# silence-tang/GaussianIP

Measured on AMD Instinct MI355X. Metric: raster_fwd_bwd_mpix_per_s, higher is better.
Workload: dtype f32; 1 GPU; BASELINE.json configs[1]: 100000 Gaussians (synthetic human surface, SMPL-X-style init), 1024x1024, 4 views per optimizer step, raster forward+backward; gaussians=100000, height=1024, width=1024, prewarm_steps=0, repeats=11, full=False, sh_degree=0, dist_world_size=1, gpus_visible=1, parallelism=1 GPU

## Files before the change

### gaussianip_amd/_lib.py

```python
import ctypes
import os

_HERE = os.path.dirname(os.path.abspath(__file__))
LIB_DIR = os.path.join(_HERE, "lib")

GIP_MAX_VIEWS = 16
GIP_RECORD_BYTES = 64
GIP_PARTIAL_FLOATS = 12
GIP_OK = 0

_vp = ctypes.c_void_p


class GipRasterConfig(ctypes.Structure):
    _fields_ = [("P", ctypes.c_int32), ("V", ctypes.c_int32), ("H", ctypes.c_int32), ("W", ctypes.c_int32),
                ("sh_degree", ctypes.c_int32), ("sh_coeffs", ctypes.c_int32), ("prefiltered", ctypes.c_int32),
                ("debug", ctypes.c_int32), ("scale_modifier", ctypes.c_float),
                ("tanfovx", ctypes.c_float * GIP_MAX_VIEWS), ("tanfovy", ctypes.c_float * GIP_MAX_VIEWS),
                ("capacity", ctypes.c_uint64), ("exact_lists", ctypes.c_int32), ("forward_only", ctypes.c_int32),
                ("sh_scalar", ctypes.c_int32), ("antialiasing", ctypes.c_int32)]


class GipRasterInputs(ctypes.Structure):
    _fields_ = [(n, _vp) for n in ("means3D", "shs", "colors_precomp", "opacities", "scales", "rotations",
# ... 33 lines not shown

call_counts = {}


class _Counted:

    def __init__(self, lib):
        self._lib = lib
        self._wrapped = {}

    def __getattr__(self, name):
        w = self._wrapped.get(name)
        if w is None:
            fn = getattr(self._lib, name)

            names = (name, name.replace("_buckets", "")) if name.startswith("gip_raster_") and "_buckets" in name else (name,)

            def w(*args, _fn=fn, _names=names):
                for n in _names:
                    call_counts[n] = call_counts.get(n, 0) + 1
                return _fn(*args)
            self._wrapped[name] = w
        return w


def raster_lib():
    global _raster
    if _raster is None:
        path = os.path.join(LIB_DIR, os.environ.get("GIP_RASTER_LIB", "libgip_raster.so"))
        if not os.path.exists(path):
            raise _missing("libgip_raster.so")
# ... 20 lines not shown
        lib.gip_raster_backward_profiled.argtypes = lib.gip_raster_backward.argtypes + [ctypes.POINTER(ctypes.c_float)]
        _u32 = ctypes.c_uint32
        lib.gip_raster_state_bytes_buckets.restype = ctypes.c_size_t
        lib.gip_raster_state_bytes_buckets.argtypes = [ctypes.POINTER(GipRasterConfig), _u32]
        lib.gip_raster_state_layout_buckets.restype = ctypes.c_int
        lib.gip_raster_state_layout_buckets.argtypes = [ctypes.POINTER(GipRasterConfig), _u32, ctypes.POINTER(GipRasterStateLayout),
                                                        ctypes.POINTER(ctypes.c_size_t)]
        lib.gip_raster_forward_buckets.restype = ctypes.c_int
        lib.gip_raster_forward_buckets.argtypes = lib.gip_raster_forward.argtypes + [_u32]
        lib.gip_raster_backward_buckets.restype = ctypes.c_int
        lib.gip_raster_backward_buckets.argtypes = lib.gip_raster_backward.argtypes + [_u32]
        lib.gip_raster_forward_buckets_profiled.restype = ctypes.c_int
        lib.gip_raster_forward_buckets_profiled.argtypes = lib.gip_raster_forward.argtypes + [_u32, ctypes.POINTER(ctypes.c_float)]
        lib.gip_raster_backward_buckets_profiled.restype = ctypes.c_int
        lib.gip_raster_backward_buckets_profiled.argtypes = lib.gip_raster_backward.argtypes + [_u32, ctypes.POINTER(ctypes.c_float)]
        lib.gip_raster_read_header.restype = ctypes.c_int
        lib.gip_raster_read_header.argtypes = [_vp, _vp, _vp]
        lib.gip_raster_mark_visible.restype = ctypes.c_int
        lib.gip_raster_mark_visible.argtypes = [ctypes.c_int32, _vp, _vp, _vp, _vp, _vp]
        _raster = _Counted(lib)
    return _raster


def knn_lib():
    global _knn
    if _knn is None:
        path = os.path.join(LIB_DIR, "libgip_knn.so")
        if not os.path.exists(path):
            raise _missing("libgip_knn.so")
        lib = ctypes.CDLL(path)
# ... 379 lines not shown
        lib.gip_softmax_rows_backward_f16.argtypes = [_vp, _vp, ctypes.c_int64, ctypes.c_int32, ctypes.c_float, _vp]
        lib.gip_scale_cast_f16.restype = ctypes.c_int
        lib.gip_scale_cast_f16.argtypes = [_vp, _vp, ctypes.c_float, _vp, ctypes.c_int64, _vp]
        _nn = _Counted(lib)
    return _nn


def status_string(rc):
    return raster_lib().gip_status_string(int(rc)).decode()


RASTER_SYMBOLS = ["gip_abi_version", "gip_status_string", "gip_raster_state_bytes", "gip_raster_scratch_bytes",
                  "gip_raster_state_layout", "gip_raster_forward", "gip_raster_backward", "gip_raster_read_header",
                  "gip_raster_mark_visible", "gip_raster_forward_profiled", "gip_raster_backward_profiled",
                  "gip_raster_state_bytes_buckets", "gip_raster_state_layout_buckets", "gip_raster_forward_buckets",
                  "gip_raster_backward_buckets", "gip_raster_forward_buckets_profiled", "gip_raster_backward_buckets_profiled"]
FIELD_SYMBOLS = ["gip_field_workspace_size", "gip_density_field", "gip_surface_count", "gip_surface_emit"]
SAMPLE_SYMBOLS = ["gip_field_sample_workspace_size", "gip_field_sample"]
TEXTURE_SYMBOLS = ["gip_texture_bake_workspace_size", "gip_texture_bake"]
TEXTURE_PROJECT_SYMBOLS = ["gip_texture_project"]
MESH_SYMBOLS = ["gip_mesh_raster_workspace_size", "gip_mesh_rasterize", "gip_mesh_interpolate", "gip_mesh_interpolate_backward",
                "gip_mesh_texture", "gip_mesh_texture_backward", "gip_mesh_shade", "gip_mesh_shade_backward"]
MESH_GRAD_SYMBOLS = ["gip_mesh_rasterize_backward", "gip_mesh_interpolate_backward_rast", "gip_mesh_shade_backward_rast", "gip_mesh_antialias",
                     "gip_mesh_antialias_backward"]
MESH_MIP_SYMBOLS = ["gip_mesh_rast_db", "gip_mesh_interpolate_da", "gip_mesh_interpolate_da_backward", "gip_mesh_mip_levels",
                    "gip_mesh_mip_build", "gip_mesh_mip_fold", "gip_mesh_texture_mip", "gip_mesh_texture_mip_backward"]
MESH_CLEAN_SYMBOLS = ["gip_mesh_components_rounds", "gip_mesh_component_stats", "gip_mesh_cluster_keys", "gip_mesh_cluster_count",
                      "gip_mesh_cluster_place"]
MESH_GEOM_SYMBOLS = ["gip_mesh_geometry_workspace_size", "gip_mesh_vertex_normals", "gip_mesh_vertex_normals_backward",
                     "gip_mesh_laplacian_loss", "gip_mesh_laplacian_loss_backward", "gip_mesh_normal_consistency",
                     "gip_mesh_normal_consistency_backward"]
# ... 10 lines not shown
```

### gaussianip_amd/csrc/api.hip

```cpp
#include <string.h>

#include "gip_internal.h"

static inline size_t align256(size_t x) { return (x + 255) & ~(size_t)255; }

static_assert(offsetof(GipRasterConfig, antialiasing) == 188 && sizeof(GipRasterConfig) == 192, "GipRasterConfig layout");

static bool sh_mfma_path(const GipRasterConfig* c) { return c->sh_coeffs > 0 && c->sh_degree >= 1 && c->V >= 2 && !c->sh_scalar; }

static bool valid_config(const GipRasterConfig* c) {
  if (!c) return false;
  if (c->P < 0 || c->V < 1 || c->V > GIP_MAX_VIEWS || c->H < 1 || c->W < 1) return false;
  if (c->sh_degree < 0 || c->sh_degree > 3) return false;
  if (c->capacity < 1 || c->capacity > 0xfffffff0ull) return false;
  if ((c->H + GIP_TILE - 1) / GIP_TILE > 0xffff || (c->W + GIP_TILE - 1) / GIP_TILE > 0xffff) return false;
  return true;
}

extern "C" int gip_abi_version(void) { return GIP_ABI_VERSION; }

extern "C" const char* gip_status_string(int status) {
  switch (status) {
    case GIP_OK: return "ok";
    case GIP_ERR_BAD_ARGUMENT: return "bad argument (null pointer, or not exactly one of shs/colors_precomp and scales+rotations/cov3D_precomp)";
// ... 96 lines not shown
  p.tile_cursor = (uint32_t*)(b + L.tile_cursor);
  p.tile_count_b = (uint32_t*)(b + L.tile_count_b);
  p.inst_slot = (uint32_t*)(b + L.inst_slot);
  p.block_sums = (uint32_t*)(b + L.block_sums);
  p.block_offset = (uint32_t*)(b + L.block_offset);
  p.keys = (unsigned long long*)(b + (bucket_keys ? bucket_keys : L.keys));
  p.n_contrib = (uint32_t*)(b + L.n_contrib);
  p.final_T = (float*)(b + L.final_T);
  p.tile_order = (uint32_t*)(b + L.tile_order);
  p.seg_start = (uint32_t*)(b + L.seg_start);
  p.ckpt_start = (uint32_t*)(b + L.ckpt_start);
  p.seg_tile = (uint32_t*)(b + L.seg_tile);
  p.checkpoints = (float*)(b + L.checkpoints);
  p.sh_colors = (float*)(b + L.sh_colors);
  p.host_header = nullptr;
  return p;
}

static int prepare(const GipRasterConfig* cfg, const GipRasterInputs* in, void* state, size_t state_bytes, uint32_t bucket_stride,
                   GipRasterStateLayout* L, GipKernelParams* kp, GipStatePtrs* st) {
  size_t bucket_keys = 0;
  if (gip_raster_state_layout_buckets(cfg, bucket_stride, L, &bucket_keys) != GIP_OK) return GIP_ERR_BAD_ARGUMENT;
  if (state_bytes < L->total) return GIP_ERR_BUFFER_TOO_SMALL;
  fill_params(cfg, *L, kp);
  kp->bucket_stride = bucket_stride;
  if (!in->shs) kp->sh_mfma = 0;
  *st = state_ptrs(state, *L, bucket_stride ? bucket_keys : 0);
  return GIP_OK;
}

// ... 39 lines not shown
    if (!ok || hipStreamSynchronize(s) != hipSuccess) rc = GIP_ERR_HIP;
    for (int i = 0; i < GIP_NUM_STAGES; i++) {
      if (rc == GIP_OK && used[i]) {
        float ms = 0.f;
        if (hipEventElapsedTime(&ms, ev[2 * i], ev[2 * i + 1]) != hipSuccess) rc = GIP_ERR_HIP;
        out[i] = ms;
      }
    }
    for (int i = 0; i < created; i++) (void)hipEventDestroy(ev[i]);
    return rc;
  }
};
}

static int forward_impl(const GipRasterConfig* cfg, const GipRasterInputs* in, const GipRasterOutputs* out,
                        void* state, size_t state_bytes, void* stream, float* times, uint32_t bucket_stride) {
  if (!valid_config(cfg)) return cfg && (cfg->V > GIP_MAX_VIEWS || cfg->sh_degree > 3) ? GIP_ERR_UNSUPPORTED : GIP_ERR_BAD_ARGUMENT;
  int rc = check_inputs(cfg, in);
  if (rc != GIP_OK) return rc;
  if (!out || !out->color || !out->radii || !out->depth || !out->alpha || !state) return GIP_ERR_BAD_ARGUMENT;
  GipRasterStateLayout L;
  GipKernelParams kp;
  GipStatePtrs st;
  rc = prepare(cfg, in, state, state_bytes, bucket_stride, &L, &kp, &st);
  if (rc != GIP_OK) return rc;
  st.host_header = out->host_header;
  hipStream_t s = (hipStream_t)stream;
  StageTimer tm(s, times);

  tm.begin(GIP_STAGE_CLEAR);
  HIP_TRY(hipMemsetAsync((char*)state + L.header, 0, L.tile_start - L.header, s));
  tm.end(GIP_STAGE_CLEAR);
  if (cfg->P > 0) {
    tm.begin(GIP_STAGE_PREPROCESS);
    if (kp.sh_mfma) gip_launch_sh_forward_mfma(kp, *in, st.sh_colors, s);
    gip_launch_preprocess(kp, *in, out->radii, st, s);
    tm.end(GIP_STAGE_PREPROCESS);
    LAUNCH_CHECK();
  }
  tm.begin(GIP_STAGE_SCAN);
  gip_launch_scan(kp, st, s);
  tm.end(GIP_STAGE_SCAN);
  LAUNCH_CHECK();
  if (cfg->P > 0) {
    if (!bucket_stride) {
      tm.begin(GIP_STAGE_SCATTER);
      gip_launch_scatter(kp, st, s);
// ... 13 lines not shown
}

extern "C" int gip_raster_forward(const GipRasterConfig* cfg, const GipRasterInputs* in, const GipRasterOutputs* out,
                                  void* state, size_t state_bytes, void* stream) {
  return forward_impl(cfg, in, out, state, state_bytes, stream, nullptr, 0);
}
extern "C" int gip_raster_forward_buckets(const GipRasterConfig* cfg, const GipRasterInputs* in, const GipRasterOutputs* out,
                                          void* state, size_t state_bytes, void* stream, uint32_t bucket_stride) {
  return forward_impl(cfg, in, out, state, state_bytes, stream, nullptr, bucket_stride);
}
extern "C" int gip_raster_forward_buckets_profiled(const GipRasterConfig* cfg, const GipRasterInputs* in, const GipRasterOutputs* out,
                                                   void* state, size_t state_bytes, void* stream, uint32_t bucket_stride,
                                                   float* times_ms) {
  if (!times_ms) return GIP_ERR_BAD_ARGUMENT;
  return forward_impl(cfg, in, out, state, state_bytes, stream, times_ms, bucket_stride);
}
extern "C" int gip_raster_forward_profiled(const GipRasterConfig* cfg, const GipRasterInputs* in, const GipRasterOutputs* out,
                                           void* state, size_t state_bytes, void* stream, float* times_ms) {
  if (!times_ms) return GIP_ERR_BAD_ARGUMENT;
  return forward_impl(cfg, in, out, state, state_bytes, stream, times_ms, 0);
}

static int backward_impl(const GipRasterConfig* cfg, const GipRasterInputs* in, const GipRasterGradsIn* gin,
                         const void* state, size_t state_bytes, void* scratch, size_t scratch_bytes,
                         const GipRasterGradsOut* gout, void* stream, float* times, uint32_t bucket_stride) {
  if (!valid_config(cfg)) return GIP_ERR_BAD_ARGUMENT;
  int rc = check_inputs(cfg, in);
  if (rc != GIP_OK) return rc;
  if (!gin || !gin->alpha || !gin->color || !gin->depth || !gout || !state || !scratch) return GIP_ERR_BAD_ARGUMENT;
  if (cfg->forward_only) return GIP_ERR_BAD_ARGUMENT;
// ... 60 lines not shown
```

### gaussianip_amd/csrc/binning.hip

```cpp
#include "gip_internal.h"
#include "tile_sort_assign.h"

#define SCAN_THREADS 1024
#define SCAN_WAVES (SCAN_THREADS / 64)
#define SCAN_CHUNK SCAN_THREADS
#define SCAN_FIN 32

__device__ __forceinline__ uint32_t nseg_of(uint32_t count) { return (count + GIP_SEGMENT - 1) / GIP_SEGMENT; }

#define ORDER_CLASSES 6
__device__ __forceinline__ int class_of(uint32_t c) {
  return c >= 2048 ? 0 : c >= 1024 ? 1 : c >= 512 ? 2 : c >= 128 ? 3 : c >= 1 ? 4 : 5;
}

__device__ __forceinline__ uint32_t block_excl_scan(uint32_t v, uint32_t* s_w, uint32_t* total) {
  const int lane = threadIdx.x & 63, wave = threadIdx.x >> 6;
  const uint32_t incl = gip_wave_incl_scan_u32(v);
  __syncthreads();
  if (lane == 63) s_w[wave] = incl;
  __syncthreads();
  uint32_t base = 0, tot = 0;
#pragma unroll
  for (int w = 0; w < SCAN_WAVES; w++) { const uint32_t x = s_w[w]; base += w < wave ? x : 0u; tot += x; }
  *total = tot;
  return base + incl - v;
}

__device__ __forceinline__ uint32_t wave_sum_u32(uint32_t v) {
#pragma unroll
  for (int d = 32; d >= 1; d >>= 1) v += (uint32_t)__shfl_xor((int)v, d, 64);
  return v;
}

__global__ void __launch_bounds__(SCAN_THREADS)
gip_scan_kernel(GipKernelParams kp, const uint32_t* __restrict__ tile_count, const uint32_t* __restrict__ tile_count_b,
                uint32_t* __restrict__ tile_start,
                uint32_t* __restrict__ seg_start, uint32_t* __restrict__ ckpt_start,
                const uint32_t* __restrict__ block_sums, uint32_t* __restrict__ block_offset,
                uint32_t* __restrict__ tile_order, GipRasterHeader* __restrict__ header, uint32_t* __restrict__ host_header,
                uint32_t* __restrict__ inst_offset) {
  __shared__ uint32_t s_w[SCAN_WAVES];
  __shared__ uint32_t s_acc[2][3 + ORDER_CLASSES];
  __shared__ uint32_t s_max;
  __shared__ uint32_t s_cls[ORDER_CLASSES][SCAN_WAVES];
  const int n = kp.V * kp.T;
  const int n_chunks = (n + SCAN_CHUNK - 1) / SCAN_CHUNK;
  const int tid = threadIdx.x, lane = tid & 63, wave = tid >> 6;
  const int nb_chunks = kp.V * kp.nblk > 0 ? (kp.V * kp.nblk + SCAN_CHUNK - 1) / SCAN_CHUNK : 1;
  if ((int)blockIdx.x >= n_chunks + nb_chunks) {
    __shared__ uint32_t s_fin[SCAN_FIN];
    const int nb = kp.V * kp.nblk;
    const int j0 = ((int)blockIdx.x - n_chunks - nb_chunks) * SCAN_FIN;
    uint32_t before = 0;
    for (int i = tid; i < j0; i += SCAN_THREADS) before += block_sums[i];
    before = wave_sum_u32(before);
    if (tid == 0) s_max = 0u;
    __syncthreads();
// ... 22 lines not shown
      uint32_t v8[8];
#pragma unroll
      for (int u = 0; u < 8; u++) { const int i = i0 + u * SCAN_THREADS; v8[u] = i < c0 ? block_sums[i] : 0u; }
#pragma unroll
      for (int u = 0; u < 8; u++) before += v8[u];
    }
    before = wave_sum_u32(before);
    if (tid == 0) s_max = 0u;
    __syncthreads();
    if (lane == 0) atomicAdd(&s_max, before);
    __syncthreads();
    const uint32_t base = s_max;
    const int i = c0 + tid;
    const uint32_t v = i < nb ? block_sums[i] : 0u;
    uint32_t total;
    const uint32_t e = block_excl_scan(v, s_w, &total);
    if (i < nb) block_offset[i] = base + e;
    if (c0 + SCAN_CHUNK >= nb && tid == 0) block_offset[nb] = base + total;
    return;
  }
  const int chunk0 = (int)blockIdx.x * SCAN_CHUNK;
  if (tid < 2 * (3 + ORDER_CLASSES)) (&s_acc[0][0])[tid] = 0u;
  if (tid == 0) s_max = 0u;
  __syncthreads();
  uint32_t b_c = 0, b_s = 0, b_k = 0, t_c = 0, t_s = 0, t_k = 0, mx = 0;
  uint32_t b_cls[ORDER_CLASSES], t_cls[ORDER_CLASSES];
#pragma unroll
  for (int c = 0; c < ORDER_CLASSES; c++) { b_cls[c] = 0; t_cls[c] = 0; }
  for (int i0 = wave * 64; i0 < n; i0 += 8 * SCAN_THREADS) {
    uint32_t va[8], vb[8];
#pragma unroll
    for (int u = 0; u < 8; u++) {
      const int i = i0 + u * SCAN_THREADS + lane;
      va[u] = i < n ? tile_count[i] : 0u;
      vb[u] = i < n ? tile_count_b[i] : 0u;
    }
#pragma unroll
    for (int u = 0; u < 8; u++) {
      const int g0 = i0 + u * SCAN_THREADS;
      if (g0 >= n) break;
      const int i = g0 + lane;
      const uint32_t c = va[u] + vb[u], a = nseg_of(c), k = a ? a - 1 : 0;
      const int cls = i < n ? class_of(c) : -1;
      const bool before = g0 < chunk0;
      t_c += c; t_s += a; t_k += k;
      mx = c > mx ? c : mx;
      if (before) { b_c += c; b_s += a; b_k += k; }
#pragma unroll
      for (int q = 0; q < ORDER_CLASSES; q++) {
        const uint32_t m = (uint32_t)__popcll(__ballot(cls == q));
        t_cls[q] += m;
        if (before) b_cls[q] += m;
      }
    }
  }
  b_c = wave_sum_u32(b_c); b_s = wave_sum_u32(b_s); b_k = wave_sum_u32(b_k);
  t_c = wave_sum_u32(t_c); t_s = wave_sum_u32(t_s); t_k = wave_sum_u32(t_k);
  mx = gip_wave_max_u32(mx);
  if (lane == 0) {
    atomicAdd(&s_acc[0][0], b_c); atomicAdd(&s_acc[0][1], b_s); atomicAdd(&s_acc[0][2], b_k);
    atomicAdd(&s_acc[1][0], t_c); atomicAdd(&s_acc[1][1], t_s); atomicAdd(&s_acc[1][2], t_k);
#pragma unroll
    for (int q = 0; q < ORDER_CLASSES; q++) { atomicAdd(&s_acc[0][3 + q], b_cls[q]); atomicAdd(&s_acc[1][3 + q], t_cls[q]); }
    atomicMax(&s_max, mx);
  }
  __syncthreads();
  const int i = chunk0 + tid;
  uint32_t c = 0;
  if (i < n) c = tile_count[i] + tile_count_b[i];
  const uint32_t a = nseg_of(c), k = a ? a - 1 : 0;
  uint32_t tot;
  const uint32_t e_c = block_excl_scan(c, s_w, &tot);
  const uint32_t e_s = block_excl_scan(a, s_w, &tot);
  const uint32_t e_k = block_excl_scan(k, s_w, &tot);
  if (i < n) {
    tile_start[i] = s_acc[0][0] + e_c;
    seg_start[i] = s_acc[0][1] + e_s;
    ckpt_start[i] = s_acc[0][2] + e_k;
  }
  const int cls = i < n ? class_of(c) : -1;
  uint32_t rank = 0;
#pragma unroll
  for (int q = 0; q < ORDER_CLASSES; q++) {
    const unsigned long long m = __ballot(cls == q);
    if (cls == q) rank = (uint32_t)__popcll(m & ((1ull << lane) - 1ull));
    if (lane == 0) s_cls[q][wave] = (uint32_t)__popcll(m);
  }
  __syncthreads();
  if (cls >= 0) {
    uint32_t pos = rank + s_acc[0][3 + cls];
#pragma unroll
    for (int q = 0; q < ORDER_CLASSES; q++) pos += q < cls ? s_acc[1][3 + q] : 0u;
    for (int w = 0; w < wave; w++) pos += s_cls[cls][w];
    tile_order[pos] = (uint32_t)i;
  }
  if (blockIdx.x == 0 && tid == 0) {
    const uint32_t total = s_acc[1][0];
    tile_start[n] = total; seg_start[n] = s_acc[1][1]; ckpt_start[n] = s_acc[1][2];
    const uint32_t n0 = s_acc[1][3], n1 = s_acc[1][4], n2 = s_acc[1][5], n3 = s_acc[1][6], n4 = s_acc[1][7];
    header->class_end[1] = n0;
    header->class_end[2] = n0 + n1;
    header->class_end[0] = n0 + n1 + n2;
    header->class_end[3] = n0 + n1 + n2 + n3 + n4;
    header->abi_version = GIP_ABI_VERSION;
    header->num_rendered = total;
    const uint32_t over = (total > kp.capacity || (kp.bucket_stride && s_max > kp.bucket_stride)) ? 1u : 0u;
    header->overflow = over;
    header->max_tile_count = s_max;
    header->reserved[0] = kp.bucket_stride;
    header->num_segments = s_acc[1][1];
    header->num_checkpoints = s_acc[1][2];
    if (host_header) {
      host_header[0] = GIP_ABI_VERSION; host_header[1] = total;
      host_header[2] = over; host_header[3] = s_max; host_header[4] = kp.bucket_stride;
    }
  }
}

void gip_launch_scan(const GipKernelParams& kp, GipStatePtrs st, hipStream_t s) {
  const int n = kp.V * kp.T, nb = kp.V * kp.nblk;
  const int n_chunks = (n + SCAN_CHUNK - 1) / SCAN_CHUNK, b_chunks = nb > 0 ? (nb + SCAN_CHUNK - 1) / SCAN_CHUNK : 1;
  const int f_chunks = kp.bucket_stride ? (nb + SCAN_FIN - 1) / SCAN_FIN : 0;
  hipLaunchKernelGGL(gip_scan_kernel, dim3(n_chunks + b_chunks + f_chunks), dim3(SCAN_THREADS), 0, s, kp, st.tile_count, st.tile_count_b, st.tile_start,
                     st.seg_start, st.ckpt_start, st.block_sums, st.block_offset, st.tile_order, st.header, st.host_header,
                     st.inst_offset);
}

__global__ void __launch_bounds__(GIP_BLOCK)
gip_scatter_kernel(GipKernelParams kp, const GipRecord* __restrict__ records, const uint32_t* __restrict__ tile_start,
                   const uint32_t* __restrict__ tile_count, uint32_t* __restrict__ tile_cursor,
                   const uint32_t* __restrict__ inst_slot, const uint32_t* __restrict__ block_offset,
                   uint32_t* __restrict__ inst_offset, unsigned long long* __restrict__ keys) {
  const int v = blockIdx.y;
  const int idx = blockIdx.x * GIP_BLOCK + threadIdx.x;
  uint32_t tiles = 0, rmin = 0, rmax = 0, dbits = 0, tmask = 0;
  if (idx < kp.P) {
    const uint4* rp = reinterpret_cast<const uint4*>(records + (size_t)v * kp.P + idx);
    const uint4 q0 = rp[0], q1 = rp[1], q3 = rp[3];
    dbits = q0.z; tiles = q1.w; rmin = q3.x; rmax = q3.y; tmask = q3.w;
  }
// ... 288 lines not shown
      for (int r = 0; r < 8; r++) { const uint32_t i = base + r * 64 + lane; if (i < n) s[padk(i)] = v[r]; }
    } else {
      wave_store<8>(a, n, base, lane, v);
    }
  }
  __syncthreads();
  const uint32_t nm = multi ? n : 0u;
  merge_level<8>(s, nm, 512, ltid);
  merge_level<8>(s, nm, 1024, ltid);
  for (uint32_t i = ltid; i < nm; i += 256) a[i] = s[padk(i)];
}

__global__ void __launch_bounds__(LONG_THREADS)
gip_tile_sort_kernel(GipKernelParams kp, GipRasterHeader* __restrict__ header, const uint32_t* __restrict__ tile_order,
                     const uint32_t* __restrict__ tile_start, const uint32_t* __restrict__ seg_start,
                     uint32_t* __restrict__ seg_tile, unsigned long long* __restrict__ keys) {
  extern __shared__ __attribute__((aligned(16))) unsigned long long s_long[];
  __shared__ uint32_t s_pos;
  const GipSortAssign as = gip_sort_assign(gridDim.x, header->class_end[1], header->class_end[0], header->class_end[3]);
  const uint32_t end_a = as.end_a, end_m = as.end_m, end_b = as.end_b;
  const int lane = threadIdx.x & 63;
  const uint32_t wave = threadIdx.x >> 6, q = threadIdx.x >> 8;
  for (uint32_t pos = gip_sort_a_pos(as, blockIdx.x); pos < end_a;) {
    const uint32_t t = tile_order[pos];
    const uint32_t start = tile_start[t];
    const uint32_t n = gip_list_len(kp, start, tile_start[t + 1]);
    if (n > 0) {
      unsigned long long* a = keys + gip_list_base(kp, t, start);
      write_seg_tiles<LONG_THREADS>(kp, seg_start, seg_tile, t, n);
      if (n > LONG_CHUNK) sort_beyond_lds(a, n, s_long);
      else if (n > 1) lds_sort<LONG_THREADS>(s_long, n, a, a);
    }
    if (end_a <= as.a_first) break;
// ... 66 lines not shown
    }
  }
}

void gip_launch_tile_sort(const GipKernelParams& kp, GipStatePtrs st, hipStream_t s) {
  static int wgs = 0;
  constexpr size_t lds = (size_t)PADK_SLOTS(LONG_CHUNK) * sizeof(unsigned long long);
  if (!wgs) {
    (void)hipFuncSetAttribute((const void*)gip_tile_sort_kernel, hipFuncAttributeMaxDynamicSharedMemorySize, (int)lds);
    int dev = 0, cus = 0;
    if (hipGetDevice(&dev) != hipSuccess || hipDeviceGetAttribute(&cus, hipDeviceAttributeMultiprocessorCount, dev) != hipSuccess || cus < 1)
      cus = 256;
    wgs = cus;
  }
  hipLaunchKernelGGL(gip_tile_sort_kernel, dim3(wgs), dim3(LONG_THREADS), lds, s, kp, st.header, st.tile_order,
                     st.tile_start, st.seg_start, st.seg_tile, st.keys);
}
```

### gaussianip_amd/csrc/gip_internal.h

```cpp
#pragma once
#include <hip/hip_runtime.h>
#include <stdint.h>

#include "../../include/gip_raster.h"

#define GIP_BLOCK 256
#define GIP_WAVE 64
#define GIP_NEAR 0.2f
#define GIP_ALPHA_MIN (1.0f / 255.0f)
#define GIP_ALPHA_MAX 0.99f
#define GIP_T_MIN 0.0001f

struct __attribute__((aligned(16))) GipRecord {
  float x, y, depth, opacity;
  float ca, cb, cc; uint32_t tiles;
  float r, g, b; int32_t radius;
  uint32_t rmin, rmax, clamped, tmask;
};

#define GIP_MASK_TILES 32
__host__ __device__ inline bool gip_rect_has(uint32_t tmask, int area, int k) { return area > GIP_MASK_TILES || ((tmask >> k) & 1u); }
__host__ __device__ inline int gip_rect_rank(uint32_t tmask, int area, int k) {
  return area > GIP_MASK_TILES ? k : __builtin_popcount(tmask & ((1u << k) - 1u));
}
// ... 14 lines not shown
  uint32_t seg_capacity;
  uint32_t ckpt_capacity;
  int exact_lists;
  int forward_only;
  int sh_mfma;
  int antialiasing;
  uint32_t bucket_stride;
  GipViewConst view[GIP_MAX_VIEWS];
};

struct GipStatePtrs {
  GipRasterHeader* header;
  GipRecord* records;
  uint32_t* inst_offset;
  uint32_t* tile_count;
  uint32_t* tile_start;
  uint32_t* tile_cursor;
  uint32_t* tile_count_b;
  uint32_t* inst_slot;
  uint32_t* block_sums;
  uint32_t* block_offset;
  unsigned long long* keys;
  uint32_t* n_contrib;
  float* final_T;
  uint32_t* tile_order;
  uint32_t* seg_start;
  uint32_t* ckpt_start;
  uint32_t* seg_tile;
  float* checkpoints;
  uint32_t* host_header;
// ... 47 lines not shown
```

### gaussianip_amd/csrc/preprocess.hip

```cpp
#include "gip_internal.h"

#define SH_C0 0.28209479177387814f
#define SH_C1 0.4886025119029199f
__device__ static const float SH_C2[5] = {1.0925484305920792f, -1.0925484305920792f, 0.31539156525252005f,
                                          -1.0925484305920792f, 0.5462742152960396f};
__device__ static const float SH_C3[7] = {-0.5900435899266435f, 2.890611442640554f, -0.4570457994644658f,
                                          0.3731763325901154f, -0.4570457994644658f, 1.445305721320277f,
                                          -0.5900435899266435f};

__device__ __forceinline__ float ndc2pix(float v, int S) { return ((v + 1.0f) * S - 1.0f) * 0.5f; }

__device__ __forceinline__ float sh_channel(int deg, const float* __restrict__ sh, int ch, float x, float y, float z) {
#define SH(k) sh[(k) * 3 + ch]
  float res = SH_C0 * SH(0);
  if (deg > 0) {
    res = res - SH_C1 * y * SH(1) + SH_C1 * z * SH(2) - SH_C1 * x * SH(3);
    if (deg > 1) {
      float xx = x * x, yy = y * y, zz = z * z, xy = x * y, yz = y * z, xz = x * z;
      res = res + SH_C2[0] * xy * SH(4) + SH_C2[1] * yz * SH(5) + SH_C2[2] * (2.0f * zz - xx - yy) * SH(6) +
            SH_C2[3] * xz * SH(7) + SH_C2[4] * (xx - yy) * SH(8);
      if (deg > 2) {
        res = res + SH_C3[0] * y * (3.0f * xx - yy) * SH(9) + SH_C3[1] * xy * z * SH(10) +
              SH_C3[2] * y * (4.0f * zz - xx - yy) * SH(11) + SH_C3[3] * z * (2.0f * zz - 3.0f * xx - 3.0f * yy) * SH(12) +
              SH_C3[4] * x * (4.0f * zz - xx - yy) * SH(13) + SH_C3[5] * z * (xx - yy) * SH(14) +
// ... 3 lines not shown
  }
#undef SH
  return res;
}

#define PRE_THREADS 1024
__global__ void __launch_bounds__(PRE_THREADS)
gip_preprocess_kernel(GipKernelParams kp, const float* __restrict__ means3D, const float* __restrict__ shs,
                      const float* __restrict__ colors_precomp, const float* __restrict__ opacities,
                      const float* __restrict__ scales, const float* __restrict__ rotations,
                      const float* __restrict__ cov3D_precomp, const float* __restrict__ viewmatrix,
                      const float* __restrict__ projmatrix, const float* __restrict__ camposs,
                      int32_t* __restrict__ radii, GipRecord* __restrict__ records,
                      uint32_t* __restrict__ tile_count, uint32_t* __restrict__ tile_count_b,
                      uint32_t* __restrict__ inst_slot, uint32_t* __restrict__ block_sums,
                      GipRasterHeader* __restrict__ header, const float* __restrict__ sh_colors,
                      unsigned long long* __restrict__ bucket_keys, uint32_t* __restrict__ inst_offset) {
  const int v = blockIdx.y;
  const int idx = blockIdx.x * PRE_THREADS + threadIdx.x;
  const float* view = viewmatrix + 16 * v;
  const float* proj = projmatrix + 16 * v;
  const float* campos = camposs + 3 * v;
  const float tanx = kp.view[v].tanfovx, tany = kp.view[v].tanfovy;
  const float fx = kp.view[v].focal_x, fy = kp.view[v].focal_y;
  const int W = kp.W, H = kp.H;

  GipRecord rec;
  rec.x = rec.y = rec.depth = rec.opacity = 0.f;
  rec.ca = rec.cb = rec.cc = 0.f; rec.tiles = 0;
  rec.r = rec.g = rec.b = 0.f; rec.radius = 0;
  rec.rmin = rec.rmax = rec.clamped = 0; rec.tmask = 0xffffffffu;
// ... 261 lines not shown
  __syncthreads();
  if (kp.bucket_stride && idx < kp.P) {
    uint32_t pre = incl - rec.tiles;
    for (int w = wave & ~(GIP_BLOCK / 64 - 1); w < wave; w++) pre += s_sum[w];
    inst_offset[(size_t)v * kp.P + idx] = pre;
  }
  if (threadIdx.x < PRE_SUB) {
    const int blk = blockIdx.x * PRE_SUB + threadIdx.x;
    const int w0 = threadIdx.x * (GIP_BLOCK / 64);
    if (blk < kp.nblk) block_sums[(size_t)v * kp.nblk + blk] = s_sum[w0] + s_sum[w0 + 1] + s_sum[w0 + 2] + s_sum[w0 + 3];
  }
  if (threadIdx.x == 0) {
    uint32_t nv = 0;
#pragma unroll
    for (int w = 0; w < PRE_WAVES; w++) nv += s_vis[w];
    if (nv) atomicAdd(&header->num_visible, nv);
  }
}

void gip_launch_preprocess(const GipKernelParams& kp, const GipRasterInputs& in, int32_t* radii, GipStatePtrs st, hipStream_t s) {
  dim3 grid((kp.nblk + PRE_THREADS / GIP_BLOCK - 1) / (PRE_THREADS / GIP_BLOCK), kp.V), block(PRE_THREADS);
  hipLaunchKernelGGL(gip_preprocess_kernel, grid, block, 0, s, kp, in.means3D, in.shs, in.colors_precomp, in.opacities,
                     in.scales, in.rotations, in.cov3D_precomp, in.viewmatrix, in.projmatrix, in.campos, radii,
                     st.records, st.tile_count, st.tile_count_b, st.inst_slot, st.block_sums, st.header,
                     kp.sh_mfma ? st.sh_colors : nullptr, st.keys, st.inst_offset);
}

__global__ void __launch_bounds__(GIP_BLOCK)
gip_mark_visible_kernel(int P, const float* __restrict__ means3D, const float* __restrict__ view, uint8_t* __restrict__ present) {
  const int idx = blockIdx.x * GIP_BLOCK + threadIdx.x;
  if (idx >= P) return;
  const float z = view[2] * means3D[3 * idx] + view[6] * means3D[3 * idx + 1] + view[10] * means3D[3 * idx + 2] + view[14];
  present[idx] = z > GIP_NEAR ? 1 : 0;
}
void gip_launch_mark_visible(int P, const float* means3D, const float* view, uint8_t* present, hipStream_t s) {
  hipLaunchKernelGGL(gip_mark_visible_kernel, dim3((P + GIP_BLOCK - 1) / GIP_BLOCK), dim3(GIP_BLOCK), 0, s, P, means3D, view, present);
}
```

### gaussianip_amd/rasterizer.py

```python
import ctypes
import os
import warnings
from typing import NamedTuple, Optional, Sequence

import torch

from . import _lib


class GaussianRasterizationSettings(NamedTuple):
    image_height: int
    image_width: int
    tanfovx: float
    tanfovy: float
    bg: torch.Tensor
    scale_modifier: float
    viewmatrix: torch.Tensor
    projmatrix: torch.Tensor
    sh_degree: int
    campos: torch.Tensor
    prefiltered: bool
    debug: bool
    antialiasing: bool = False

# ... 50 lines not shown


def _bucket_key(key):
    return key + (_exact_lists(),)


def _pick_stride(bkey, V, H, W):
    last = _bucket_hint.get(bkey)
    if last is None or not _buckets_enabled():
        return 0
    S = bucket_stride(last)
    T = ((H + 15) // 16) * ((W + 15) // 16)
    return S if V * T * S * 8 <= _bucket_budget() else 0


_dummy = {}


def _ptr(t):
    if t is None:
        return None
    if t.numel() == 0:
        d = _dummy.get(t.device)
        if d is None:
            d = _dummy[t.device] = torch.zeros(64, dtype=torch.float32, device=t.device)
        return ctypes.c_void_p(d.data_ptr())
    return ctypes.c_void_p(t.data_ptr())


def _f32c(t, name):
# ... 1 lines not shown
        return None
    if not t.is_cuda:
        raise ValueError("%s must be a CUDA/HIP tensor (the rasterizer has no CPU path)" % name)
    if t.dtype != torch.float32 or not t.is_contiguous():
        t = t.float().contiguous()
    return t


class _Plan:
    means3D = shs = colors_precomp = opacities = scales = rotations = cov3D_precomp = None
    viewmatrix = projmatrix = campos = bg = None
    P = V = H = W = sh_degree = M = 0
    scale_modifier, tanfovx, tanfovy = 1.0, (), ()
    prefiltered = debug = antialiasing = False
    bucket_stride = capacity = 0
    cfg = state = host_header = None
    header_slot = -1
    dense_first_call = False
    pending = None
    num_rendered, overflowed = None, False


def _make_config(plan, capacity, forward_only):
    cfg = _lib.GipRasterConfig()
    cfg.P, cfg.V, cfg.H, cfg.W = plan.P, plan.V, plan.H, plan.W
    cfg.sh_degree, cfg.sh_coeffs = plan.sh_degree, plan.M
    cfg.prefiltered, cfg.debug = int(plan.prefiltered), int(plan.debug)
    cfg.scale_modifier = plan.scale_modifier
    cfg.tanfovx[:plan.V], cfg.tanfovy[:plan.V] = plan.tanfovx, plan.tanfovy
    cfg.capacity = int(capacity)
# ... 27 lines not shown
    def mk(like, *shape):
        return None if like is None else torch.empty(shape, dtype=torch.float32, device=dev)

    g = dict(means3D=mk(plan.means3D, P, 3), means2D=mk(plan.means3D, V, P, 3), shs=mk(plan.shs, P, max(M, 1), 3),
             colors_precomp=mk(plan.colors_precomp, P, 3), opacities=mk(plan.opacities, P, 1), scales=mk(plan.scales, P, 3),
             rotations=mk(plan.rotations, P, 4), cov3D_precomp=mk(plan.cov3D_precomp, P, 6))
    gout = _lib.GipRasterGradsOut(_ptr(g["means3D"]), _ptr(g["means2D"]), _ptr(g["shs"]), _ptr(g["colors_precomp"]),
                                  _ptr(g["opacities"]), _ptr(g["scales"]), _ptr(g["rotations"]), _ptr(g["cov3D_precomp"]))
    return scratch, g, gout


def _launch_forward(plan, outs, times=None):
    lib = _lib.raster_lib()
    cfg, ins, stream = _marshal(plan)
    args = (ctypes.byref(cfg), ctypes.byref(ins), ctypes.byref(outs), _ptr(plan.state), plan.state.numel(), stream, plan.bucket_stride)
    rc = lib.gip_raster_forward_buckets(*args) if times is None else lib.gip_raster_forward_buckets_profiled(*args, times)
    _check(rc, "gip_raster_forward")


def _launch_backward(plan, gin, scratch, gout, times=None):
    lib = _lib.raster_lib()
    cfg, ins, stream = _marshal(plan)
    args = (ctypes.byref(cfg), ctypes.byref(ins), ctypes.byref(gin), _ptr(plan.state), plan.state.numel(), _ptr(scratch), scratch.numel(),
            ctypes.byref(gout), stream, plan.bucket_stride)
    rc = lib.gip_raster_backward_buckets(*args) if times is None else lib.gip_raster_backward_buckets_profiled(*args, times)
    _check(rc, "gip_raster_backward")


def _run_forward(plan, capacity, forward_only=False):
    dev = plan.means3D.device
    plan.capacity = capacity
# ... 289 lines not shown
        return st[off:off + nbytes].view(dtype).reshape(shape)

    tile_start = view(L.tile_start, V * T + 1, torch.int32, (V * T + 1,))
    if S:
        buckets = view(bucket_off.value, V * T * S, torch.int64, (V * T * S,))
        ts = tile_start.long()
        n = min(int(ts[-1]), int(plan.capacity))
        pos = torch.arange(n, device=st.device)
        vt = torch.searchsorted(ts[1:].contiguous(), pos, right=True)
        off = pos - ts[vt]
        keys = torch.zeros(int(plan.capacity), dtype=torch.int64, device=st.device)
        ok = off < S
        keys[:n][ok] = buckets[(vt * S + off)[ok]]
    else:
        keys = view(L.keys, int(plan.capacity), torch.int64, (int(plan.capacity),))
    return dict(
        header=view(L.header, 16, torch.int32, (16,)),
        records=view(L.records, V * P * 16, torch.float32, (V, P, 16)),
        records_u32=view(L.records, V * P * 16, torch.int32, (V, P, 16)),
        inst_offset=view(L.inst_offset, V * P, torch.int32, (V, P)),
        tile_count=view(L.tile_count, V * T, torch.int32, (V, T)),
        tile_start=tile_start,
        keys=keys,
        n_contrib=view(L.n_contrib, V * H * W, torch.int32, (V, H, W)),
        seg_start=view(L.seg_start, V * T + 1, torch.int32, (V * T + 1,)),
        seg_tile=view(L.seg_tile, (L.checkpoints - L.seg_tile) // 4, torch.int32, ((L.checkpoints - L.seg_tile) // 4,)),
        tiles_x=L.tiles_x, tiles_y=L.tiles_y)


def forward_with_state(means3D, opacities, settings_list, shs=None, colors_precomp=None, scales=None, rotations=None,
                       cov3D_precomp=None):
    _validate(shs, colors_precomp, scales, rotations, cov3D_precomp)
    plan = _build_plan(means3D, shs, colors_precomp, opacities, scales, rotations, cov3D_precomp, list(settings_list))
    outs = _forward_with_policy(plan, False)
    return outs, plan

# ... 24 lines not shown
```

### include/gip_raster.h

```cpp
#ifndef GIP_RASTER_H
#define GIP_RASTER_H

#include <stddef.h>
#include <stdint.h>

#ifdef __cplusplus
extern "C" {
#endif

#define GIP_ABI_VERSION 4
#define GIP_TILE 16
#define GIP_MAX_VIEWS 16
#define GIP_RECORD_BYTES 64
#define GIP_PARTIAL_FLOATS 12
#ifndef GIP_SEGMENT
#define GIP_SEGMENT 64
#endif
#define GIP_SLOTS 8
#define GIP_CKPT_FLOATS 5

enum {
  GIP_OK = 0,
  GIP_ERR_BAD_ARGUMENT = 1,
  GIP_ERR_BUFFER_TOO_SMALL = 2,
// ... 126 lines not shown
int    gip_raster_state_layout_buckets(const GipRasterConfig* cfg, uint32_t bucket_stride, GipRasterStateLayout* out,
                                       size_t* bucket_keys );
int gip_raster_forward_buckets(const GipRasterConfig* cfg, const GipRasterInputs* in, const GipRasterOutputs* out,
                               void* state, size_t state_bytes, void* stream, uint32_t bucket_stride);
int gip_raster_backward_buckets(const GipRasterConfig* cfg, const GipRasterInputs* in, const GipRasterGradsIn* gin,
                                const void* state, size_t state_bytes, void* scratch, size_t scratch_bytes,
                                const GipRasterGradsOut* gout, void* stream, uint32_t bucket_stride);
int gip_raster_forward_buckets_profiled(const GipRasterConfig* cfg, const GipRasterInputs* in, const GipRasterOutputs* out,
                                        void* state, size_t state_bytes, void* stream, uint32_t bucket_stride,
                                        float* times_ms );
int gip_raster_backward_buckets_profiled(const GipRasterConfig* cfg, const GipRasterInputs* in, const GipRasterGradsIn* gin,
                                         const void* state, size_t state_bytes, void* scratch, size_t scratch_bytes,
                                         const GipRasterGradsOut* gout, void* stream, uint32_t bucket_stride,
                                         float* times_ms );

int gip_raster_read_header(const void* state, GipRasterHeader* host_header, void* stream);

int gip_raster_mark_visible(int32_t P, const float* means3D, const float* viewmatrix, const float* projmatrix,
                            uint8_t* present, void* stream);

#ifdef __cplusplus
}
#endif
#endif
```

Before: 9452 Mpix/s.

## Replace per-forward state memset with self-clearing persistent tile counters

```diff
diff --git a/gaussianip_amd/_lib.py b/gaussianip_amd/_lib.py
--- a/gaussianip_amd/_lib.py
+++ b/gaussianip_amd/_lib.py
@@ -71,7 +71,8 @@
         if w is None:
             fn = getattr(self._lib, name)
 
-            names = (name, name.replace("_buckets", "")) if name.startswith("gip_raster_") and "_buckets" in name else (name,)
+            plain = name.replace("_buckets", "").replace("_counters", "")
+            names = (name, plain) if name.startswith("gip_raster_") and plain != name else (name,)
 
             def w(*args, _fn=fn, _names=names):
                 for n in _names:
@@ -122,6 +123,10 @@
         lib.gip_raster_forward_buckets_profiled.argtypes = lib.gip_raster_forward.argtypes + [_u32, ctypes.POINTER(ctypes.c_float)]
         lib.gip_raster_backward_buckets_profiled.restype = ctypes.c_int
         lib.gip_raster_backward_buckets_profiled.argtypes = lib.gip_raster_backward.argtypes + [_u32, ctypes.POINTER(ctypes.c_float)]
+        lib.gip_raster_forward_counters.restype = ctypes.c_int
+        lib.gip_raster_forward_counters.argtypes = lib.gip_raster_forward.argtypes + [_u32, _vp]
+        lib.gip_raster_forward_counters_profiled.restype = ctypes.c_int
+        lib.gip_raster_forward_counters_profiled.argtypes = lib.gip_raster_forward.argtypes + [_u32, _vp, ctypes.POINTER(ctypes.c_float)]
         lib.gip_raster_read_header.restype = ctypes.c_int
         lib.gip_raster_read_header.argtypes = [_vp, _vp, _vp]
         lib.gip_raster_mark_visible.restype = ctypes.c_int
@@ -531,7 +536,8 @@
                   "gip_raster_state_layout", "gip_raster_forward", "gip_raster_backward", "gip_raster_read_header",
                   "gip_raster_mark_visible", "gip_raster_forward_profiled", "gip_raster_backward_profiled",
                   "gip_raster_state_bytes_buckets", "gip_raster_state_layout_buckets", "gip_raster_forward_buckets",
-                  "gip_raster_backward_buckets", "gip_raster_forward_buckets_profiled", "gip_raster_backward_buckets_profiled"]
+                  "gip_raster_backward_buckets", "gip_raster_forward_buckets_profiled", "gip_raster_backward_buckets_profiled",
+                  "gip_raster_forward_counters", "gip_raster_forward_counters_profiled"]
 FIELD_SYMBOLS = ["gip_field_workspace_size", "gip_density_field", "gip_surface_count", "gip_surface_emit"]
 SAMPLE_SYMBOLS = ["gip_field_sample_workspace_size", "gip_field_sample"]
 TEXTURE_SYMBOLS = ["gip_texture_bake_workspace_size", "gip_texture_bake"]
diff --git a/gaussianip_amd/csrc/api.hip b/gaussianip_amd/csrc/api.hip
--- a/gaussianip_amd/csrc/api.hip
+++ b/gaussianip_amd/csrc/api.hip
@@ -134,6 +134,7 @@
   p.checkpoints = (float*)(b + L.checkpoints);
   p.sh_colors = (float*)(b + L.sh_colors);
   p.host_header = nullptr;
+  p.counters = nullptr;
   return p;
 }
 
@@ -203,7 +204,8 @@
 }
 
 static int forward_impl(const GipRasterConfig* cfg, const GipRasterInputs* in, const GipRasterOutputs* out,
-                        void* state, size_t state_bytes, void* stream, float* times, uint32_t bucket_stride) {
+                        void* state, size_t state_bytes, void* stream, float* times, uint32_t bucket_stride,
+                        uint32_t* counters = nullptr) {
   if (!valid_config(cfg)) return cfg && (cfg->V > GIP_MAX_VIEWS || cfg->sh_degree > 3) ? GIP_ERR_UNSUPPORTED : GIP_ERR_BAD_ARGUMENT;
   int rc = check_inputs(cfg, in);
   if (rc != GIP_OK) return rc;
@@ -217,9 +219,14 @@
   hipStream_t s = (hipStream_t)stream;
   StageTimer tm(s, times);
 
-  tm.begin(GIP_STAGE_CLEAR);
-  HIP_TRY(hipMemsetAsync((char*)state + L.header, 0, L.tile_start - L.header, s));
-  tm.end(GIP_STAGE_CLEAR);
+  if (counters && bucket_stride) {
+    st.counters = counters;
+    st.tile_count = counters;
+  } else {
+    tm.begin(GIP_STAGE_CLEAR);
+    HIP_TRY(hipMemsetAsync((char*)state + L.header, 0, L.tile_start - L.header, s));
+    tm.end(GIP_STAGE_CLEAR);
+  }
   if (cfg->P > 0) {
     tm.begin(GIP_STAGE_PREPROCESS);
     if (kp.sh_mfma) gip_launch_sh_forward_mfma(kp, *in, st.sh_colors, s);
@@ -263,6 +270,16 @@
                                                    float* times_ms) {
   if (!times_ms) return GIP_ERR_BAD_ARGUMENT;
   return forward_impl(cfg, in, out, state, state_bytes, stream, times_ms, bucket_stride);
+}
+extern "C" int gip_raster_forward_counters(const GipRasterConfig* cfg, const GipRasterInputs* in, const GipRasterOutputs* out,
+                                           void* state, size_t state_bytes, void* stream, uint32_t bucket_stride, uint32_t* counters) {
+  return forward_impl(cfg, in, out, state, state_bytes, stream, nullptr, bucket_stride, counters);
+}
+extern "C" int gip_raster_forward_counters_profiled(const GipRasterConfig* cfg, const GipRasterInputs* in, const GipRasterOutputs* out,
+                                                    void* state, size_t state_bytes, void* stream, uint32_t bucket_stride,
+                                                    uint32_t* counters, float* times_ms) {
+  if (!times_ms) return GIP_ERR_BAD_ARGUMENT;
+  return forward_impl(cfg, in, out, state, state_bytes, stream, times_ms, bucket_stride, counters);
 }
 extern "C" int gip_raster_forward_profiled(const GipRasterConfig* cfg, const GipRasterInputs* in, const GipRasterOutputs* out,
                                            void* state, size_t state_bytes, void* stream, float* times_ms) {
diff --git a/gaussianip_amd/csrc/binning.hip b/gaussianip_amd/csrc/binning.hip
--- a/gaussianip_amd/csrc/binning.hip
+++ b/gaussianip_amd/csrc/binning.hip
@@ -32,15 +32,16 @@
   return v;
 }
 
+template <bool TWO_COUNTS>
 __global__ void __launch_bounds__(SCAN_THREADS)
 gip_scan_kernel(GipKernelParams kp, const uint32_t* __restrict__ tile_count, const uint32_t* __restrict__ tile_count_b,
                 uint32_t* __restrict__ tile_start,
                 uint32_t* __restrict__ seg_start, uint32_t* __restrict__ ckpt_start,
                 const uint32_t* __restrict__ block_sums, uint32_t* __restrict__ block_offset,
                 uint32_t* __restrict__ tile_order, GipRasterHeader* __restrict__ header, uint32_t* __restrict__ host_header,
-                uint32_t* __restrict__ inst_offset) {
-  __shared__ uint32_t s_w[SCAN_WAVES];
-  __shared__ uint32_t s_acc[2][3 + ORDER_CLASSES];
+                uint32_t* __restrict__ inst_offset, const uint32_t* __restrict__ counters) {
+  __shared__ unsigned long long s_w[SCAN_WAVES];
+  __shared__ uint32_t s_acc[2][2 + ORDER_CLASSES];
   __shared__ uint32_t s_max;
   __shared__ uint32_t s_cls[ORDER_CLASSES][SCAN_WAVES];
   const int n = kp.V * kp.T;
@@ -93,38 +94,46 @@
     const int i = c0 + tid;
     const uint32_t v = i < nb ? block_sums[i] : 0u;
     uint32_t total;
-    const uint32_t e = block_excl_scan(v, s_w, &total);
+    const uint32_t e = block_excl_scan(v, reinterpret_cast<uint32_t*>(s_w), &total);
     if (i < nb) block_offset[i] = base + e;
     if (c0 + SCAN_CHUNK >= nb && tid == 0) block_offset[nb] = base + total;
     return;
   }
   const int chunk0 = (int)blockIdx.x * SCAN_CHUNK;
-  if (tid < 2 * (3 + ORDER_CLASSES)) (&s_acc[0][0])[tid] = 0u;
+  const uint32_t n_vis = (counters && blockIdx.x == 0 && tid == 0) ? counters[n] : 0u;
+  if (tid < 2 * (2 + ORDER_CLASSES)) (&s_acc[0][0])[tid] = 0u;
   if (tid == 0) s_max = 0u;
   __syncthreads();
-  uint32_t b_c = 0, b_s = 0, b_k = 0, t_c = 0, t_s = 0, t_k = 0, mx = 0;
+  uint32_t b_c = 0, b_s = 0, t_c = 0, t_s = 0, mx = 0;
   uint32_t b_cls[ORDER_CLASSES], t_cls[ORDER_CLASSES];
 #pragma unroll
   for (int c = 0; c < ORDER_CLASSES; c++) { b_cls[c] = 0; t_cls[c] = 0; }
-  for (int i0 = wave * 64; i0 < n; i0 += 8 * SCAN_THREADS) {
-    uint32_t va[8], vb[8];
+  uint32_t c_own = 0;
+  uint32_t va[8], vb[8];
+  auto load8 = [&](int i0, uint32_t (&a8)[8], uint32_t (&b8)[8]) __attribute__((always_inline)) {
 #pragma unroll
     for (int u = 0; u < 8; u++) {
       const int i = i0 + u * SCAN_THREADS + lane;
-      va[u] = i < n ? tile_count[i] : 0u;
-      vb[u] = i < n ? tile_count_b[i] : 0u;
-    }
+      a8[u] = i < n ? tile_count[i] : 0u;
+      b8[u] = (TWO_COUNTS && i < n) ? tile_count_b[i] : 0u;
+    }
+  };
+  load8(wave * 64, va, vb);
+  for (int i0 = wave * 64; i0 < n; i0 += 8 * SCAN_THREADS) {
+    uint32_t na[8], nb[8];
+    load8(i0 + 8 * SCAN_THREADS, na, nb);
 #pragma unroll
     for (int u = 0; u < 8; u++) {
       const int g0 = i0 + u * SCAN_THREADS;
       if (g0 >= n) break;
       const int i = g0 + lane;
-      const uint32_t c = va[u] + vb[u], a = nseg_of(c), k = a ? a - 1 : 0;
+      const uint32_t c = va[u] + vb[u], a = nseg_of(c);
       const int cls = i < n ? class_of(c) : -1;
       const bool before = g0 < chunk0;
-      t_c += c; t_s += a; t_k += k;
+      if (g0 == chunk0 + wave * 64) c_own = c;
+      t_c += c; t_s += a;
       mx = c > mx ? c : mx;
-      if (before) { b_c += c; b_s += a; b_k += k; }
+      if (before) { b_c += c; b_s += a; }
 #pragma unroll
       for (int q = 0; q < ORDER_CLASSES; q++) {
         const uint32_t m = (uint32_t)__popcll(__ballot(cls == q));
@@ -132,51 +141,59 @@
         if (before) b_cls[q] += m;
       }
     }
-  }
-  b_c = wave_sum_u32(b_c); b_s = wave_sum_u32(b_s); b_k = wave_sum_u32(b_k);
-  t_c = wave_sum_u32(t_c); t_s = wave_sum_u32(t_s); t_k = wave_sum_u32(t_k);
+#pragma unroll
+    for (int u = 0; u < 8; u++) { va[u] = na[u]; vb[u] = nb[u]; }
+  }
+  b_c = wave_sum_u32(b_c); b_s = wave_sum_u32(b_s);
+  t_c = wave_sum_u32(t_c); t_s = wave_sum_u32(t_s);
   mx = gip_wave_max_u32(mx);
   if (lane == 0) {
-    atomicAdd(&s_acc[0][0], b_c); atomicAdd(&s_acc[0][1], b_s); atomicAdd(&s_acc[0][2], b_k);
-    atomicAdd(&s_acc[1][0], t_c); atomicAdd(&s_acc[1][1], t_s); atomicAdd(&s_acc[1][2], t_k);
-#pragma unroll
-    for (int q = 0; q < ORDER_CLASSES; q++) { atomicAdd(&s_acc[0][3 + q], b_cls[q]); atomicAdd(&s_acc[1][3 + q], t_cls[q]); }
+    atomicAdd(&s_acc[0][0], b_c); atomicAdd(&s_acc[0][1], b_s);
+    atomicAdd(&s_acc[1][0], t_c); atomicAdd(&s_acc[1][1], t_s);
+#pragma unroll
+    for (int q = 0; q < ORDER_CLASSES; q++) { atomicAdd(&s_acc[0][2 + q], b_cls[q]); atomicAdd(&s_acc[1][2 + q], t_cls[q]); }
     atomicMax(&s_max, mx);
   }
-  __syncthreads();
   const int i = chunk0 + tid;
-  uint32_t c = 0;
-  if (i < n) c = tile_count[i] + tile_count_b[i];
-  const uint32_t a = nseg_of(c), k = a ? a - 1 : 0;
-  uint32_t tot;
-  const uint32_t e_c = block_excl_scan(c, s_w, &tot);
-  const uint32_t e_s = block_excl_scan(a, s_w, &tot);
-  const uint32_t e_k = block_excl_scan(k, s_w, &tot);
+  const uint32_t c = c_own, a = nseg_of(c);
+  const uint32_t i_c = gip_wave_incl_scan_u32(c), i_s = gip_wave_incl_scan_u32(a);
+  if (lane == 63) s_w[wave] = ((unsigned long long)i_c << 32) | i_s;
+  const int cls = i < n ? class_of(c) : -1;
+  const unsigned long long lanes_below = (1ull << lane) - 1ull;
+  uint32_t rank = 0, empty_below = 0;
+#pragma unroll
+  for (int q = 0; q < ORDER_CLASSES; q++) {
+    const unsigned long long m = __ballot(cls == q);
+    if (cls == q) rank = (uint32_t)__popcll(m & lanes_below);
+    if (q == ORDER_CLASSES - 1) empty_below = (uint32_t)__popcll(m & lanes_below);
+    if (lane == 0) s_cls[q][wave] = (uint32_t)__popcll(m);
+  }
+  __syncthreads();
+  unsigned long long w_before = 0;
+  uint32_t empty_before = empty_below;
+#pragma unroll
+  for (int w = 0; w < SCAN_WAVES; w++) {
+    w_before += w < wave ? s_w[w] : 0ull;
+    empty_before += w < wave ? s_cls[ORDER_CLASSES - 1][w] : 0u;
+  }
   if (i < n) {
+    const uint32_t e_c = (uint32_t)(w_before >> 32) + i_c - c, e_s = (uint32_t)w_before + i_s - a;
     tile_start[i] = s_acc[0][0] + e_c;
     seg_start[i] = s_acc[0][1] + e_s;
-    ckpt_start[i] = s_acc[0][2] + e_k;
-  }
-  const int cls = i < n ? class_of(c) : -1;
-  uint32_t rank = 0;
-#pragma unroll
-  for (int q = 0; q < ORDER_CLASSES; q++) {
-    const unsigned long long m = __ballot(cls == q);
-    if (cls == q) rank = (uint32_t)__popcll(m & ((1ull << lane) - 1ull));
-    if (lane == 0) s_cls[q][wave] = (uint32_t)__popcll(m);
-  }
-  __syncthreads();
+    ckpt_start[i] = (s_acc[0][1] + e_s) - (((uint32_t)chunk0 - s_acc[0][2 + ORDER_CLASSES - 1]) + ((uint32_t)tid - empty_before));
+  }
   if (cls >= 0) {
-    uint32_t pos = rank + s_acc[0][3 + cls];
-#pragma unroll
-    for (int q = 0; q < ORDER_CLASSES; q++) pos += q < cls ? s_acc[1][3 + q] : 0u;
+    uint32_t pos = rank + s_acc[0][2 + cls];
+#pragma unroll
+    for (int q = 0; q < ORDER_CLASSES; q++) pos += q < cls ? s_acc[1][2 + q] : 0u;
     for (int w = 0; w < wave; w++) pos += s_cls[cls][w];
     tile_order[pos] = (uint32_t)i;
   }
   if (blockIdx.x == 0 && tid == 0) {
     const uint32_t total = s_acc[1][0];
-    tile_start[n] = total; seg_start[n] = s_acc[1][1]; ckpt_start[n] = s_acc[1][2];
-    const uint32_t n0 = s_acc[1][3], n1 = s_acc[1][4], n2 = s_acc[1][5], n3 = s_acc[1][6], n4 = s_acc[1][7];
+    const uint32_t n_seg = s_acc[1][1], n_ckpt = n_seg - ((uint32_t)n - s_acc[1][2 + ORDER_CLASSES - 1]);
+    tile_start[n] = total; seg_start[n] = n_seg; ckpt_start[n] = n_ckpt;
+    const uint32_t n0 = s_acc[1][2], n1 = s_acc[1][3], n2 = s_acc[1][4], n3 = s_acc[1][5], n4 = s_acc[1][6];
     header->class_end[1] = n0;
     header->class_end[2] = n0 + n1;
     header->class_end[0] = n0 + n1 + n2;
@@ -187,8 +204,13 @@
     header->overflow = over;
     header->max_tile_count = s_max;
     header->reserved[0] = kp.bucket_stride;
-    header->num_segments = s_acc[1][1];
-    header->num_checkpoints = s_acc[1][2];
+    header->num_segments = n_seg;
+    header->num_checkpoints = n_ckpt;
+    if (counters) {
+      header->num_visible = n_vis;
+      header->sort_cursor = 0; header->sort_cursor_m = 0;
+      header->reserved[1] = 0; header->reserved[2] = 0;
+    }
     if (host_header) {
       host_header[0] = GIP_ABI_VERSION; host_header[1] = total;
       host_header[2] = over; host_header[3] = s_max; host_header[4] = kp.bucket_stride;
@@ -200,9 +222,13 @@
   const int n = kp.V * kp.T, nb = kp.V * kp.nblk;
   const int n_chunks = (n + SCAN_CHUNK - 1) / SCAN_CHUNK, b_chunks = nb > 0 ? (nb + SCAN_CHUNK - 1) / SCAN_CHUNK : 1;
   const int f_chunks = kp.bucket_stride ? (nb + SCAN_FIN - 1) / SCAN_FIN : 0;
-  hipLaunchKernelGGL(gip_scan_kernel, dim3(n_chunks + b_chunks + f_chunks), dim3(SCAN_THREADS), 0, s, kp, st.tile_count, st.tile_count_b, st.tile_start,
-                     st.seg_start, st.ckpt_start, st.block_sums, st.block_offset, st.tile_order, st.header, st.host_header,
-                     st.inst_offset);
+  const dim3 grid(n_chunks + b_chunks + f_chunks), block(SCAN_THREADS);
+  if (kp.bucket_stride)
+    hipLaunchKernelGGL(gip_scan_kernel<false>, grid, block, 0, s, kp, st.tile_count, st.tile_count_b, st.tile_start, st.seg_start,
+                       st.ckpt_start, st.block_sums, st.block_offset, st.tile_order, st.header, st.host_header, st.inst_offset, st.counters);
+  else
+    hipLaunchKernelGGL(gip_scan_kernel<true>, grid, block, 0, s, kp, st.tile_count, st.tile_count_b, st.tile_start, st.seg_start,
+                       st.ckpt_start, st.block_sums, st.block_offset, st.tile_order, st.header, st.host_header, st.inst_offset, st.counters);
 }
 
 __global__ void __launch_bounds__(GIP_BLOCK)
@@ -521,9 +547,13 @@
 __global__ void __launch_bounds__(LONG_THREADS)
 gip_tile_sort_kernel(GipKernelParams kp, GipRasterHeader* __restrict__ header, const uint32_t* __restrict__ tile_order,
                      const uint32_t* __restrict__ tile_start, const uint32_t* __restrict__ seg_start,
-                     uint32_t* __restrict__ seg_tile, unsigned long long* __restrict__ keys) {
+                     uint32_t* __restrict__ seg_tile, unsigned long long* __restrict__ keys, uint32_t* __restrict__ counters) {
   extern __shared__ __attribute__((aligned(16))) unsigned long long s_long[];
   __shared__ uint32_t s_pos;
+  if (counters) {
+    const uint32_t n1 = (uint32_t)(kp.V * kp.T) + 1u;
+    for (uint32_t i = blockIdx.x * LONG_THREADS + threadIdx.x; i < n1; i += gridDim.x * LONG_THREADS) counters[i] = 0u;
+  }
   const GipSortAssign as = gip_sort_assign(gridDim.x, header->class_end[1], header->class_end[0], header->class_end[3]);
   const uint32_t end_a = as.end_a, end_m = as.end_m, end_b = as.end_b;
   const int lane = threadIdx.x & 63;
@@ -620,5 +650,5 @@
     wgs = cus;
   }
   hipLaunchKernelGGL(gip_tile_sort_kernel, dim3(wgs), dim3(LONG_THREADS), lds, s, kp, st.header, st.tile_order,
-                     st.tile_start, st.seg_start, st.seg_tile, st.keys);
-}
+                     st.tile_start, st.seg_start, st.seg_tile, st.keys, st.counters);
+}
diff --git a/gaussianip_amd/csrc/gip_internal.h b/gaussianip_amd/csrc/gip_internal.h
--- a/gaussianip_amd/csrc/gip_internal.h
+++ b/gaussianip_amd/csrc/gip_internal.h
@@ -52,6 +52,7 @@
   GipRecord* records;
   uint32_t* inst_offset;
   uint32_t* tile_count;
+  uint32_t* counters;
   uint32_t* tile_start;
   uint32_t* tile_cursor;
   uint32_t* tile_count_b;
diff --git a/gaussianip_amd/csrc/preprocess.hip b/gaussianip_amd/csrc/preprocess.hip
--- a/gaussianip_amd/csrc/preprocess.hip
+++ b/gaussianip_amd/csrc/preprocess.hip
@@ -41,7 +41,7 @@
                       int32_t* __restrict__ radii, GipRecord* __restrict__ records,
                       uint32_t* __restrict__ tile_count, uint32_t* __restrict__ tile_count_b,
                       uint32_t* __restrict__ inst_slot, uint32_t* __restrict__ block_sums,
-                      GipRasterHeader* __restrict__ header, const float* __restrict__ sh_colors,
+                      uint32_t* __restrict__ num_visible, const float* __restrict__ sh_colors,
                       unsigned long long* __restrict__ bucket_keys, uint32_t* __restrict__ inst_offset) {
   const int v = blockIdx.y;
   const int idx = blockIdx.x * PRE_THREADS + threadIdx.x;
@@ -333,7 +333,7 @@
     uint32_t nv = 0;
 #pragma unroll
     for (int w = 0; w < PRE_WAVES; w++) nv += s_vis[w];
-    if (nv) atomicAdd(&header->num_visible, nv);
+    if (nv) atomicAdd(num_visible, nv);
   }
 }
 
@@ -341,7 +341,8 @@
   dim3 grid((kp.nblk + PRE_THREADS / GIP_BLOCK - 1) / (PRE_THREADS / GIP_BLOCK), kp.V), block(PRE_THREADS);
   hipLaunchKernelGGL(gip_preprocess_kernel, grid, block, 0, s, kp, in.means3D, in.shs, in.colors_precomp, in.opacities,
                      in.scales, in.rotations, in.cov3D_precomp, in.viewmatrix, in.projmatrix, in.campos, radii,
-                     st.records, st.tile_count, st.tile_count_b, st.inst_slot, st.block_sums, st.header,
+                     st.records, st.tile_count, st.tile_count_b, st.inst_slot, st.block_sums,
+                     st.counters ? st.counters + (size_t)kp.V * kp.T : &st.header->num_visible,
                      kp.sh_mfma ? st.sh_colors : nullptr, st.keys, st.inst_offset);
 }
 
diff --git a/gaussianip_amd/rasterizer.py b/gaussianip_amd/rasterizer.py
--- a/gaussianip_amd/rasterizer.py
+++ b/gaussianip_amd/rasterizer.py
@@ -88,6 +88,25 @@
     return S if V * T * S * 8 <= _bucket_budget() else 0
 
 
+_counter_buffers = {}
+
+
+def _clear_launch():
+    return os.environ.get("GIP_RASTER_CLEAR_LAUNCH", "0") == "1"
+
+
+def _counter_buffer(plan, stream):
+    if not plan.bucket_stride or _clear_launch():
+        return None, None
+    dev = plan.means3D.device
+    tiles = ((plan.H + 15) // 16) * ((plan.W + 15) // 16)
+    key = (dev.index if dev.index is not None else torch.cuda.current_device(), stream.value or 0, plan.V, tiles)
+    buf = _counter_buffers.get(key)
+    if buf is None:
+        buf = _counter_buffers[key] = torch.zeros(plan.V * tiles + 1, dtype=torch.int32, device=dev)
+    return key, buf
+
+
 _dummy = {}
 
 
@@ -119,6 +138,7 @@
     scale_modifier, tanfovx, tanfovy = 1.0, (), ()
     prefiltered = debug = antialiasing = False
     bucket_stride = capacity = 0
+    counters = False
     cfg = state = host_header = None
     header_slot = -1
     dense_first_call = False
@@ -176,7 +196,19 @@
     lib = _lib.raster_lib()
     cfg, ins, stream = _marshal(plan)
     args = (ctypes.byref(cfg), ctypes.byref(ins), ctypes.byref(outs), _ptr(plan.state), plan.state.numel(), stream, plan.bucket_stride)
-    rc = lib.gip_raster_forward_buckets(*args) if times is None else lib.gip_raster_forward_buckets_profiled(*args, times)
+    key, counters = _counter_buffer(plan, stream)
+    plan.counters = counters is not None
+    if counters is None:
+        rc = lib.gip_raster_forward_buckets(*args) if times is None else lib.gip_raster_forward_buckets_profiled(*args, times)
+    else:
+        args += (_ptr(counters),)
+        try:
+            rc = lib.gip_raster_forward_counters(*args) if times is None else lib.gip_raster_forward_counters_profiled(*args, times)
+        except BaseException:
+            _counter_buffers.pop(key, None)
+            raise
+        if rc != _lib.GIP_OK:
+            _counter_buffers.pop(key, None)
     _check(rc, "gip_raster_forward")
 
 
@@ -496,12 +528,16 @@
         keys[:n][ok] = buckets[(vt * S + off)[ok]]
     else:
         keys = view(L.keys, int(plan.capacity), torch.int64, (int(plan.capacity),))
+    if plan.counters:
+        tile_count = (tile_start[1:] - tile_start[:-1]).reshape(V, T)
+    else:
+        tile_count = view(L.tile_count, V * T, torch.int32, (V, T))
     return dict(
         header=view(L.header, 16, torch.int32, (16,)),
         records=view(L.records, V * P * 16, torch.float32, (V, P, 16)),
         records_u32=view(L.records, V * P * 16, torch.int32, (V, P, 16)),
         inst_offset=view(L.inst_offset, V * P, torch.int32, (V, P)),
-        tile_count=view(L.tile_count, V * T, torch.int32, (V, T)),
+        tile_count=tile_count,
         tile_start=tile_start,
         keys=keys,
         n_contrib=view(L.n_contrib, V * H * W, torch.int32, (V, H, W)),
diff --git a/include/gip_raster.h b/include/gip_raster.h
--- a/include/gip_raster.h
+++ b/include/gip_raster.h
@@ -164,6 +164,12 @@
                                          const GipRasterGradsOut* gout, void* stream, uint32_t bucket_stride,
                                          float* times_ms );
 
+int gip_raster_forward_counters(const GipRasterConfig* cfg, const GipRasterInputs* in, const GipRasterOutputs* out,
+                                void* state, size_t state_bytes, void* stream, uint32_t bucket_stride, uint32_t* counters);
+int gip_raster_forward_counters_profiled(const GipRasterConfig* cfg, const GipRasterInputs* in, const GipRasterOutputs* out,
+                                         void* state, size_t state_bytes, void* stream, uint32_t bucket_stride, uint32_t* counters,
+                                         float* times_ms );
+
 int gip_raster_read_header(const void* state, GipRasterHeader* host_header, void* stream);
 
 int gip_raster_mark_visible(int32_t P, const float* means3D, const float* viewmatrix, const float* projmatrix,
```

After: 9542 Mpix/s, median of 6. About the same (+1.0%).
